# yanyan-li/PlanarSLAM

Measured on AMD Instinct MI355X. Metric: RGB-D frames/sec (extract+match+pose-opt) @640x480; 1->8-GPU batch scaling, higher is better.
Workload: dtype u8/f64

## Files before the change

### planarslam_amd/csrc/guided.hip

```cpp
#include "common.h"
#include "match_chunk.h"
#include "ref_arith.h"

namespace planar {
namespace guided {

using namespace chunk;
using ref::Pose;

enum { MODE_FRAME = 0, MODE_MAP = 1, MODE_BOW = 2, MODE_KF = 3 };

struct Args {
    planar_frame_view f;
    planar_last_frame_view last;
    planar_map_probes mp;
    float th, nn_ratio;
    int mono, check_orientation;
    int32_t* match;
    int32_t* nmatches;
    planar_keyframe_probes kf;
    float lsf;
    int n_levels, orb_dist;
};

template <int MODE>
__device__ void resolve_chunk(ChunkLds& s, int m, const Args& a, int32_t* match, int b, const float* from_angle, const float* to_angle_f,
                              const planar_keypoint* keys, const uint8_t* observed) {
    const int lane = threadIdx.x;
    volatile uint32_t* blk = s.blocked;
    for (int q = 0; q < m; q++) {
        const int id = s.pid[q];
        const int off = s.poff[q], cnt = s.poff[q + 1] - off;
        if (id < 0 || cnt == 0) continue;
        uint32_t k1 = 0xffffffffu;
        for (int base = 0; base < cnt; base += 64) {
            const uint32_t key = unblocked_key(s, off, cnt, base + lane, -1);
            k1 = min(k1, key);
        }
        k1 = wave_min_u32_shfl(k1);
        if (k1 == 0xffffffffu) continue;
        const int bestDist = (int)(k1 >> 16), bestK = (int)(k1 & 0xffff);
        const uint32_t e1 = s.cand[off + bestK];
        const int bestIdx = e1 & 0xfff, bestLevel = (e1 >> 12) & 0xf;
        int bestDist2 = 256, bestLevel2 = -1;
        if (MODE != MODE_FRAME && MODE != MODE_KF) {
            uint32_t k2 = 0xffffffffu;
            for (int base = 0; base < cnt; base += 64) {
                const uint32_t key = unblocked_key(s, off, cnt, base + lane, bestK);
                k2 = min(k2, key);
            }
            k2 = wave_min_u32_shfl(k2);
            if (k2 != 0xffffffffu) {
                bestDist2 = (int)(k2 >> 16);
                bestLevel2 = (s.cand[off + (k2 & 0xffff)] >> 12) & 0xf;
            }
        }
        bool take;
        if (MODE == MODE_FRAME) take = bestDist <= TH_HIGH;
        else if (MODE == MODE_MAP) take = bestDist <= TH_HIGH && !(bestLevel == bestLevel2 && (float)bestDist > a.nn_ratio * (float)bestDist2);
        else if (MODE == MODE_KF) take = bestDist <= a.orb_dist;
        else take = bestDist <= TH_LOW && (float)bestDist < a.nn_ratio * (float)bestDist2;
        if (!take) continue;
        if (lane == 0) {
            match[bestIdx] = id;
            const bool now_blocked = (MODE == MODE_BOW || MODE == MODE_KF) ? true : (observed[id] != 0);
            const uint32_t w = blk[bestIdx >> 5], bit = 1u << (bestIdx & 31);
            blk[bestIdx >> 5] = now_blocked ? (w | bit) : (w & ~bit);
            s.nmatches++;
            if (MODE != MODE_MAP && a.check_orientation) {
                const float to = MODE == MODE_BOW ? to_angle_f[bestIdx] : keys[bestIdx].angle;
                const int n = s.n_ev++;
                s.ev_idx[n] = (uint16_t)bestIdx;
                s.ev_bin[n] = (uint8_t)ref::rot_bin(from_angle[id], to);
            }
        }
        __builtin_amdgcn_wave_barrier();
    }
}

template <int MODE>
__global__ __launch_bounds__(NT) void projection_kernel(Args a) {
    extern __shared__ __align__(16) uint8_t lds_raw[];
    ChunkLds& s = *(ChunkLds*)lds_raw;
    const int b = blockIdx.x, tid = threadIdx.x;
    const planar_frame_view& f = a.f;
    const int N = f.n[b];
    const planar_keypoint* keys = f.keys_un + (size_t)b * f.stride;
    const float* uR = f.u_right + (size_t)b * f.stride;
    const uint8_t* desc = f.desc + (size_t)b * f.stride * 32;
    int32_t* const match_b = a.match + (size_t)b * f.stride;

    for (int w = tid; w < MAXN / 32; w += NT) s.blocked[w] = 0;
    if (tid == 0) { s.n_ev = 0; s.nmatches = 0; }
    build_grid(s, f, keys, N);
    if (f.blocked) {
        const uint8_t* bl = f.blocked + (size_t)b * f.stride;
        for (int i = tid; i < N; i += NT)
            if (bl[i]) atomicOr(&s.blocked[i >> 5], 1u << (i & 31));
    }

    Pose P;
    bool bForward = false, bBackward = false;
    size_t po;
    int NP;
    const uint8_t *probe_desc, *observed;
    if (MODE == MODE_FRAME) {
        const float* Tl = a.last.Tcw + (size_t)b * 16;
        ref::load_pose_frame(f.Tcw + (size_t)b * 16, P);
        const float tlc2 = ref::gemm_small_row_add(Tl + 8, P.Ow, Tl[11]);
        bForward = tlc2 > f.b && !a.mono;
        bBackward = -tlc2 > f.b && !a.mono;
        po = (size_t)b * a.last.stride;
        NP = a.last.n[b];
        probe_desc = a.last.mp_desc + po * 32;
        observed = a.last.mp_observed + po;
    } else if (MODE == MODE_KF) {
        ref::load_pose_frame(f.Tcw + (size_t)b * 16, P);
        po = (size_t)b * a.kf.stride;
        NP = a.kf.n[b];
        probe_desc = a.kf.desc + po * 32;
        observed = nullptr;
    } else {
        po = (size_t)b * a.mp.stride;
        NP = a.mp.n[b];
        probe_desc = a.mp.desc + po * 32;
        observed = a.mp.observed + po;
    }
    const bool bFactor = a.th != 1.0f;
    __syncthreads();

    for (int base = 0; base < NP;) {
        const int p = base + tid;
        bool valid = false;
        float u = 0, v = 0, r = 0, ur = 0;
        int minL = -1, maxL = -1;
        if (p < NP) {
            if (MODE == MODE_FRAME) {
                if (a.last.usable[po + p]) {
                    const float* xw = a.last.xw + (po + p) * 3;
                    const float xc = ref::gemm_small_row_add(P.Rcw, xw, P.tcw[0]);
                    const float yc = ref::gemm_small_row_add(P.Rcw + 3, xw, P.tcw[1]);
                    const float zc = ref::gemm_small_row_add(P.Rcw + 6, xw, P.tcw[2]);
                    const float invzc = (float)(1.0 / (double)zc);
                    if (!(invzc < 0)) {
                        u = f.fx * xc * invzc + f.cx;
                        v = f.fy * yc * invzc + f.cy;
                        if (!(u < f.min_x || u > f.max_x) && !(v < f.min_y || v > f.max_y)) {
                            const int oct = a.last.octave[po + p];
                            r = a.th * f.scale_factors[oct];
                            if (bForward) { minL = oct; maxL = -1; }
                            else if (bBackward) { minL = 0; maxL = oct; }
                            else { minL = oct - 1; maxL = oct + 1; }
                            ur = u - f.bf * invzc;
                            valid = true;
                        }
                    }
                }
            } else if (MODE == MODE_KF) {
                if (a.kf.usable[po + p] && !(a.kf.found && a.kf.found[po + p])) {
                    const float* X = a.kf.xw + (po + p) * 3;
                    const float xc = ref::gemm_small_row_add(P.Rcw, X, P.tcw[0]);
                    const float yc = ref::gemm_small_row_add(P.Rcw + 3, X, P.tcw[1]);
                    const float zc = ref::gemm_small_row_add(P.Rcw + 6, X, P.tcw[2]);
                    const float invzc = (float)(1.0 / (double)zc);
                    u = f.fx * xc * invzc + f.cx;
                    v = f.fy * yc * invzc + f.cy;
                    if (!(u < f.min_x || u > f.max_x) && !(v < f.min_y || v > f.max_y)) {
                        const float PO[3] = {X[0] - P.Ow[0], X[1] - P.Ow[1], X[2] - P.Ow[2]};
                        const float dist3D = (float)ref::norm3(PO);
                        const float maxDistance = 1.2f * a.kf.max_dist[po + p], minDistance = 0.8f * a.kf.min_dist[po + p];
                        if (!(dist3D < minDistance || dist3D > maxDistance)) {
                            const float ratio = a.kf.max_dist[po + p] / dist3D;
                            int lvl = (int)ceilf((float)log((double)ratio) / a.lsf);
                            if (lvl < 0) lvl = 0; else if (lvl >= a.n_levels) lvl = a.n_levels - 1;
                            r = a.th * f.scale_factors[lvl];
                            minL = lvl - 1; maxL = lvl + 1;
                            valid = true;
                        }
                    }
                }
            } else {
                if (a.mp.in_view[po + p]) {
                    const int lvl = a.mp.level[po + p];
                    float rr = (double)a.mp.view_cos[po + p] > 0.998 ? 2.5f : 4.0f;
                    if (bFactor) rr *= a.th;
                    r = rr * f.scale_factors[lvl];
                    u = a.mp.proj_x[po + p]; v = a.mp.proj_y[po + p]; ur = a.mp.proj_xr[po + p];
                    minL = lvl - 1; maxL = lvl;
                    valid = true;
                }
            }
        }
        int cnt = 0;
        if (valid) frame_features_in_area<MODE != MODE_KF>(s, f, keys, uR, u, v, r, minL, maxL, ur, [&](int, int) { cnt++; });
        int total;
        const int off = ref::block_exscan<NT / 64>(cnt, s.wsum, &total);
        if (tid == 0) s.m_fit = 0;
        __syncthreads();
        const bool fits = p < NP && off + cnt <= CAND_CAP;
        if (fits) atomicAdd(&s.m_fit, 1);
        s.pid[tid] = valid ? p : -1;
        s.poff[tid] = off;
        if (tid == NT - 1) s.poff[NT] = total;
        __syncthreads();
        const int m = s.m_fit;
        if (fits && valid && cnt > 0) {
            uint32_t d[8];
            ref::load_desc(d, probe_desc + (size_t)p * 32);
            int k = off;
            frame_features_in_area<MODE != MODE_KF>(s, f, keys, uR, u, v, r, minL, maxL, ur, [&](int idx, int oct) {
                const int dist = ref::hamming256(d, desc + (size_t)idx * 32);
                s.cand[k++] = ((uint32_t)dist << 16) | ((uint32_t)(oct & 0xf) << 12) | (uint32_t)idx;
            });
        }
        __syncthreads();
        const float* from_angle = MODE == MODE_FRAME ? a.last.angle + po : MODE == MODE_KF ? a.kf.angle + po : nullptr;
        if (tid < 64) resolve_chunk<MODE>(s, m, a, match_b, b, from_angle, nullptr, keys, observed);
        __syncthreads();
        base += m;
    }
    if (MODE == MODE_FRAME && a.check_orientation) rotation_filter(s, match_b);
    if (MODE == MODE_KF && a.check_orientation) rotation_filter_ranked(s, match_b);
    __syncthreads();
    if (tid == 0) a.nmatches[b] = s.nmatches;
}

struct BowArgs {
    const int32_t *n_kf, *kf_node, *n_f, *f_node;
    const uint8_t *kf_usable, *kf_desc, *f_desc;
    const float *kf_angle, *f_angle;
    int kf_stride, f_stride;
};

struct BowLds {
    ChunkLds base;
    unsigned long long kkey[MAXN], fkey[MAXN];
};

__global__ __launch_bounds__(NT) void bow_kernel(BowArgs g, Args a) {
    extern __shared__ __align__(16) uint8_t lds_raw[];
    BowLds& L = *(BowLds*)lds_raw;
    ChunkLds& s = L.base;
    const int b = blockIdx.x, tid = threadIdx.x;
    const int NK = g.n_kf[b], NF = g.n_f[b];
    const size_t ko = (size_t)b * g.kf_stride, fo = (size_t)b * g.f_stride;
    int32_t* const match_b = a.match + fo;
    for (int w = tid; w < MAXN / 32; w += NT) s.blocked[w] = 0;
    if (tid == 0) { s.n_ev = 0; s.nmatches = 0; }
    for (int i = tid; i < NF; i += NT) match_b[i] = -1;
    int pk = 1; while (pk < NK) pk <<= 1;
    int pf = 1; while (pf < NF) pf <<= 1;
    for (int i = tid; i < pk; i += NT) {
        const int node = i < NK ? g.kf_node[ko + i] : -1;
        L.kkey[i] = node >= 0 ? ((unsigned long long)node << 12) | (unsigned)i : ~0ull;
    }
    for (int i = tid; i < pf; i += NT) {
        const int node = i < NF ? g.f_node[fo + i] : -1;
        L.fkey[i] = node >= 0 ? ((unsigned long long)node << 12) | (unsigned)i : ~0ull;
    }
    bitonic_sort_u64(L.kkey, pk);
    bitonic_sort_u64(L.fkey, pf);

    for (int base = 0; base < NK;) {
        const int p = base + tid;
        bool valid = false;
        int lo = 0, hi = 0, kf = -1;
        if (p < NK && L.kkey[p] != ~0ull) {
            kf = (int)(L.kkey[p] & 0xfff);
            if (g.kf_usable[ko + kf]) {
                const unsigned long long node = L.kkey[p] >> 12;
                int x = 0, y = NF;
                while (x < y) { const int mid = (x + y) >> 1; if ((L.fkey[mid] >> 12) < node) x = mid + 1; else y = mid; }
                lo = x; y = NF;
                while (x < y) { const int mid = (x + y) >> 1; if ((L.fkey[mid] >> 12) <= node) x = mid + 1; else y = mid; }
                hi = x;
                valid = true;
            }
        }
        const int cnt = valid ? hi - lo : 0;
        int total;
        const int off = ref::block_exscan<NT / 64>(cnt, s.wsum, &total);
        if (tid == 0) s.m_fit = 0;
        __syncthreads();
        const bool fits = p < NK && off + cnt <= CAND_CAP;
        if (fits) atomicAdd(&s.m_fit, 1);
        s.pid[tid] = valid ? kf : -1;
        s.poff[tid] = off;
        if (tid == NT - 1) s.poff[NT] = total;
        __syncthreads();
        const int m = s.m_fit;
        if (fits && cnt > 0) {
            uint32_t d[8];
            ref::load_desc(d, g.kf_desc + (ko + kf) * 32);
            for (int k = 0; k < cnt; k++) {
                const int idx = (int)(L.fkey[lo + k] & 0xfff);
                const int dist = ref::hamming256(d, g.f_desc + (fo + idx) * 32);
                s.cand[off + k] = ((uint32_t)dist << 16) | (uint32_t)idx;
            }
        }
        __syncthreads();
        if (tid < 64) resolve_chunk<MODE_BOW>(s, m, a, match_b, b, g.kf_angle + ko, g.f_angle + fo, nullptr, nullptr);
        __syncthreads();
        base += m;
    }
    if (a.check_orientation) rotation_filter(s, match_b);
    __syncthreads();
    if (tid == 0) a.nmatches[b] = s.nmatches;
}

constexpr int MAX_LINES = 1024;

struct LineArgs {
    const int32_t *n_lines, *n_ml, *ml_level;
    const planar_keyline* keylines;
    const uint8_t *ldesc, *blocked, *ml_in_view, *ml_desc, *ml_observed;
    const float *ml_proj, *ml_view_cos;
    int line_stride, ml_stride;
    float scale_factors[PLANAR_MAX_LEVELS];
    float th, nn_ratio;
    int32_t *match, *nmatches;
};

__global__ __launch_bounds__(64) void lsd_projection_kernel(LineArgs a) {
    __shared__ uint32_t blocked[MAX_LINES / 32];
    const int b = blockIdx.x, lane = threadIdx.x;
    const int NLn = a.n_lines[b], NM = a.n_ml[b];
    const size_t lo = (size_t)b * a.line_stride, mo = (size_t)b * a.ml_stride;
    const planar_keyline* kl = a.keylines + lo;
    const uint8_t* ldesc = a.ldesc + lo * 32;
    int32_t* match = a.match + lo;
    volatile uint32_t* blk = blocked;
    for (int w = lane; w < MAX_LINES / 32; w += 64) blocked[w] = 0;
    __builtin_amdgcn_wave_barrier();
    if (a.blocked)
        for (int i = lane; i < NLn; i += 64)
            if (a.blocked[lo + i]) atomicOr(&blocked[i >> 5], 1u << (i & 31));
    __builtin_amdgcn_wave_barrier();
    const bool bFactor = a.th != 1.0f;
    int nmatches = 0;
    for (int j = 0; j < NM; j++) {
        if (!a.ml_in_view[mo + j]) continue;
        const int lvl = a.ml_level[mo + j];
        if (lvl < 0 || lvl >= PLANAR_MAX_LEVELS) continue;
        float r = (double)a.ml_view_cos[mo + j] > 0.998 ? 5.0f : 8.0f;
        if (bFactor) r *= a.th;
        const float* pr = a.ml_proj + (mo + j) * 4;
        const float x1 = pr[0], y1 = pr[1], x2 = pr[2], y2 = pr[3];
        const float rr = r * a.scale_factors[lvl];
        const int minLevel = lvl - 1, maxLevel = lvl;
        const bool bCheckLevels = (minLevel > 0) || (maxLevel > 0);
        uint32_t d[8];
        ref::load_desc(d, a.ml_desc + (mo + j) * 32);
        uint32_t k1 = 0xffffffffu, k2 = 0xffffffffu;
        for (int pass = 0; pass < 2; pass++) {
            uint32_t kmin = 0xffffffffu;
            for (int base = 0; base < NLn; base += 64) {
                const int i = base + lane;
                uint32_t key = 0xffffffffu;
                if (i < NLn && !(pass == 1 && i == (int)(k1 & 0xffff))) {
                    const planar_keyline k = kl[i];
                    const double mx = 0.5 * (double)(x1 + x2) - (double)k.pt_x, my = 0.5 * (double)(y1 + y2) - (double)k.pt_y;
                    const float distance = (float)(mx * mx + my * my);
                    bool ok = !(distance > rr * rr);
                    const float slope = (y1 - y2) / (x1 - x2) - k.angle;
                    if ((double)slope > (double)rr * 0.01) ok = false;
                    if (bCheckLevels) {
                        if (k.octave < minLevel) ok = false;
                        if (maxLevel >= 0 && k.octave > maxLevel) ok = false;
                    }
                    if (ok && !((blk[i >> 5] >> (i & 31)) & 1u)) key = ((uint32_t)ref::hamming256(d, ldesc + (size_t)i * 32) << 16) | (uint32_t)i;
                }
                kmin = min(kmin, key);
            }
            kmin = wave_min_u32_shfl(kmin);
            if (pass == 0) { k1 = kmin; if (k1 == 0xffffffffu) break; } else k2 = kmin;
        }
        if (k1 == 0xffffffffu) continue;
        const int bestDist = (int)(k1 >> 16), bestIdx = (int)(k1 & 0xffff);
        const int bestLevel = kl[bestIdx].octave;
        int bestDist2 = 256, bestLevel2 = -1;
        if (k2 != 0xffffffffu) { bestDist2 = (int)(k2 >> 16); bestLevel2 = kl[k2 & 0xffff].octave; }
        if (bestDist <= TH_HIGH) {
            if (bestLevel == bestLevel2 && (float)bestDist > a.nn_ratio * (float)bestDist2) continue;
            if (lane == 0) {
                match[bestIdx] = j;
                const uint32_t w = blk[bestIdx >> 5], bit = 1u << (bestIdx & 31);
                blk[bestIdx >> 5] = a.ml_observed[mo + j] ? (w | bit) : (w & ~bit);
            }
            nmatches++;
            __builtin_amdgcn_wave_barrier();
        }
    }
    if (lane == 0) a.nmatches[b] = nmatches;
}

__global__ __launch_bounds__(64) void plane_match_kernel(const int32_t* n_planes, int pl_stride, const float* pl_coef, const float* Tcw,
                                                         int map_shared, const int32_t* n_mp, int mp_stride, const uint8_t* mp_valid,
                                                         const float* mp_coef, const int32_t* mp_npts, int pts_stride, const float* mp_pts,
                                                         float dTh, float aTh, float verTh, float parTh, int32_t* match, int32_t* ver,
                                                         int32_t* par, int32_t* nmatches) {
    const int b = blockIdx.y, i = blockIdx.x, lane = threadIdx.x;
    if (i >= n_planes[b]) return;
    const int m = map_shared ? 0 : b;
    const size_t po = (size_t)b * pl_stride + i, mo = (size_t)m * mp_stride;
    const float* T = Tcw + (size_t)b * 16;
    const float* c = pl_coef + po * 4;
    float pM[4];
    for (int r = 0; r < 4; r++) {
        const float t = T[r] * c[0] + T[4 + r] * c[1] + T[8 + r] * c[2] + T[12 + r] * c[3];
        pM[r] = (float)((double)t * 1.0);
    }
    float ldTh = dTh, lverTh = verTh, lparTh = parTh;
    bool found = false;
    int im = -1, iv = -1, ip = -1;
    const int NM = n_mp[m];
    for (int j = 0; j < NM; j++) {
        if (!mp_valid[mo + j]) continue;
        const float* pW = mp_coef + (mo + j) * 4;
        const float angle = pM[0] * pW[0] + pM[1] * pW[1] + pM[2] * pW[2];
        if (angle > aTh || angle < -aTh) {
            const float* pts = mp_pts + (mo + j) * (size_t)pts_stride * 3;
            const int np = mp_npts[mo + j];
            float res = 100.0f;
            for (int k = lane; k < np; k += 64) {
                const float dis = fabsf(pM[0] * pts[3 * k] + pM[1] * pts[3 * k + 1] + pM[2] * pts[3 * k + 2] + pM[3]);
                res = fminf(res, dis);
            }
            for (int o = 32; o >= 1; o >>= 1) res = fminf(res, __shfl_xor(res, o, 64));
            if ((double)res < (double)ldTh) { ldTh = res; im = j; found = true; continue; }
        }
        if (angle < lverTh && angle > -lverTh) { lverTh = fabsf(angle); iv = j; continue; }
        if (angle > lparTh || angle < -lparTh) { lparTh = fabsf(angle); ip = j; }
    }
    if (lane == 0) {
        if (im >= 0) match[po] = im;
        if (iv >= 0) ver[po] = iv;
        if (ip >= 0) par[po] = ip;
        if (found) atomicAdd(&nmatches[b], 1);
    }
}

__global__ __launch_bounds__(256) void frustum_points_kernel(planar_frame_view F, float lsf, int n_levels, const int32_t* __restrict__ n, int stride,
                                                             const uint8_t* __restrict__ valid, const float* __restrict__ xw,
                                                             const float* __restrict__ normal, const float* __restrict__ min_dist,
                                                             const float* __restrict__ max_dist, float limit, uint8_t* __restrict__ in_view,
                                                             float* __restrict__ proj_x, float* __restrict__ proj_y, float* __restrict__ proj_xr,
                                                             int32_t* __restrict__ level, float* __restrict__ view_cos) {
    const int b = blockIdx.y, j = blockIdx.x * 256 + threadIdx.x;
    if (j >= n[b]) return;
    const size_t o = (size_t)b * stride + j;
    in_view[o] = 0;
    if (!valid[o]) return;
    Pose P;
    ref::load_pose_frame(F.Tcw + (size_t)b * 16, P);
// ... 536 lines not shown
                       d_normal, d_min_dist, d_max_dist, viewing_cos_limit, d_in_view, d_proj, d_level, d_view_cos);
    PLANAR_HIP_CHECK(hipGetLastError());
    return PLANAR_OK;
}

int planar_is_in_frustum_lines(planar_ctx* ctx, const planar_frame_view* f, float log_scale_factor, const int32_t* n, int stride, const uint8_t* valid,
                               const double* xw6, const double* normal, const float* min_dist, const float* max_dist, float viewing_cos_limit, uint8_t* in_view,
                               float* proj, int32_t* level, float* view_cos) {
    if (int rc = check_frustum_args(ctx, f, 1, stride, n && valid && xw6 && normal && min_dist && max_dist && in_view && proj && level && view_cos)) return rc;
    PLANAR_HIP_CHECK(hipSetDevice(ctx->device));
    Stager s;
    planar_frame_view d = *f;
    const size_t B = (size_t)f->B, N = B * stride;
    s.in_field(d.Tcw, B * 16);
    const auto d_n = s.in(n, B);
    const auto d_valid = s.in(valid, N);
    const auto d_xw6 = s.in(xw6, N * 6), d_normal = s.in(normal, N * 3);
    const auto d_min = s.in(min_dist, N), d_max = s.in(max_dist, N);
    const auto d_in_view = s.inout(in_view, N);
    const auto d_proj = s.inout(proj, N * 4);
    const auto d_level = s.inout(level, N);
    const auto d_cos = s.inout(view_cos, N);
    return s.run(ctx->stream, [&] {
        return planar_is_in_frustum_lines_dev(ctx, &d, log_scale_factor, d_n, stride, d_valid, d_xw6, d_normal, d_min, d_max, viewing_cos_limit, d_in_view, d_proj, d_level, d_cos);
    });
}

int planar_search_by_bow_dev(planar_ctx* ctx, int B, const int32_t* d_n_kf, int kf_stride, const int32_t* d_kf_node, const uint8_t* d_kf_usable,
                             const float* d_kf_angle, const uint8_t* d_kf_desc, const int32_t* d_n_f, int f_stride, const int32_t* d_f_node,
                             const float* d_f_angle, const uint8_t* d_f_desc, float nn_ratio, int check_orientation, int32_t* d_match,
                             int32_t* d_nmatches) {
    if (int rc = check_bow_args(ctx, B, kf_stride, f_stride, d_n_kf && d_kf_node && d_kf_usable && d_kf_angle && d_kf_desc && d_n_f && d_f_node && d_f_angle && d_f_desc && d_match &&
                                                                 d_nmatches))
        return rc;
    static bool attr_set = false;
    if (!attr_set) {
        PLANAR_HIP_CHECK(hipFuncSetAttribute((const void*)guided::bow_kernel, hipFuncAttributeMaxDynamicSharedMemorySize, (int)sizeof(guided::BowLds)));
        attr_set = true;
    }
    guided::BowArgs g{d_n_kf, d_kf_node, d_n_f, d_f_node, d_kf_usable, d_kf_desc, d_f_desc, d_kf_angle, d_f_angle, kf_stride, f_stride};
    Args a{};
    a.nn_ratio = nn_ratio; a.check_orientation = check_orientation; a.match = d_match; a.nmatches = d_nmatches;
    hipLaunchKernelGGL(guided::bow_kernel, dim3(B), dim3(guided::NT), sizeof(guided::BowLds), ctx->stream, g, a);
    PLANAR_HIP_CHECK(hipGetLastError());
    return PLANAR_OK;
}

int planar_search_by_bow(planar_ctx* ctx, int B, const int32_t* n_kf, int kf_stride, const int32_t* kf_node, const uint8_t* kf_usable,
                         const float* kf_angle, const uint8_t* kf_desc, const int32_t* n_f, int f_stride, const int32_t* f_node,
                         const float* f_angle, const uint8_t* f_desc, float nn_ratio, int check_orientation, int32_t* match, int32_t* nmatches) {
    if (int rc = check_bow_args(ctx, B, kf_stride, f_stride, n_kf && kf_node && kf_usable && kf_angle && kf_desc && n_f && f_node && f_angle && f_desc && match && nmatches)) return rc;
    PLANAR_HIP_CHECK(hipSetDevice(ctx->device));
    Stager s;
    const size_t nb = (size_t)B, nk = nb * kf_stride, nf = nb * f_stride;
    const auto d_n_kf = s.in(n_kf, nb), d_kf_node = s.in(kf_node, nk);
    const auto d_kf_usable = s.in(kf_usable, nk);
    const auto d_kf_angle = s.in(kf_angle, nk);
    const auto d_kf_desc = s.in(kf_desc, nk * 32);
    const auto d_n_f = s.in(n_f, nb), d_f_node = s.in(f_node, nf);
    const auto d_f_angle = s.in(f_angle, nf);
    const auto d_f_desc = s.in(f_desc, nf * 32);
    const auto d_match = s.inout(match, nf), d_n = s.out(nmatches, nb);
    return s.run(ctx->stream, [&] {
        return planar_search_by_bow_dev(ctx, B, d_n_kf, kf_stride, d_kf_node, d_kf_usable, d_kf_angle, d_kf_desc, d_n_f, f_stride, d_f_node, d_f_angle, d_f_desc, nn_ratio,
                                        check_orientation, d_match, d_n);
    });
}

int planar_lsd_search_by_projection_dev(planar_ctx* ctx, int B, const int32_t* d_n_lines, int line_stride, const planar_keyline* d_keylines,
                                        const uint8_t* d_ldesc, const uint8_t* d_blocked, const int32_t* d_n_ml, int ml_stride,
                                        const uint8_t* d_ml_in_view, const float* d_ml_proj, const int32_t* d_ml_level, const float* d_ml_view_cos,
                                        const uint8_t* d_ml_desc, const uint8_t* d_ml_observed, const float* scale_factors, int n_levels, float th,
                                        float nn_ratio, int32_t* d_match, int32_t* d_nmatches) {
    if (int rc = check_lsd_projection_args(ctx, B, line_stride, ml_stride, n_levels, d_n_lines && d_keylines && d_ldesc && d_n_ml && d_ml_in_view && d_ml_proj && d_ml_level &&
                                                                                         d_ml_view_cos && d_ml_desc && d_ml_observed && scale_factors && d_match && d_nmatches))
        return rc;
    guided::LineArgs a{};
    a.n_lines = d_n_lines; a.n_ml = d_n_ml; a.ml_level = d_ml_level; a.keylines = d_keylines; a.ldesc = d_ldesc; a.blocked = d_blocked;
    a.ml_in_view = d_ml_in_view; a.ml_desc = d_ml_desc; a.ml_observed = d_ml_observed; a.ml_proj = d_ml_proj; a.ml_view_cos = d_ml_view_cos;
    a.line_stride = line_stride; a.ml_stride = ml_stride; a.th = th; a.nn_ratio = nn_ratio; a.match = d_match; a.nmatches = d_nmatches;
    for (int i = 0; i < n_levels; i++) a.scale_factors[i] = scale_factors[i];
    hipLaunchKernelGGL(guided::lsd_projection_kernel, dim3(B), dim3(64), 0, ctx->stream, a);
    PLANAR_HIP_CHECK(hipGetLastError());
    return PLANAR_OK;
}

int planar_lsd_search_by_projection(planar_ctx* ctx, int B, const int32_t* n_lines, int line_stride, const planar_keyline* keylines,
                                    const uint8_t* ldesc, const uint8_t* blocked, const int32_t* n_ml, int ml_stride, const uint8_t* ml_in_view,
                                    const float* ml_proj, const int32_t* ml_level, const float* ml_view_cos, const uint8_t* ml_desc,
                                    const uint8_t* ml_observed, const float* scale_factors, int n_levels, float th, float nn_ratio, int32_t* match,
                                    int32_t* nmatches) {
    if (int rc = check_lsd_projection_args(ctx, B, line_stride, ml_stride, n_levels, n_lines && keylines && ldesc && n_ml && ml_in_view && ml_proj && ml_level && ml_view_cos &&
                                                                                         ml_desc && ml_observed && scale_factors && match && nmatches))
        return rc;
    PLANAR_HIP_CHECK(hipSetDevice(ctx->device));
    Stager s;
    const size_t nb = (size_t)B, nl = nb * line_stride, nm = nb * ml_stride;
    const auto d_n_lines = s.in(n_lines, nb);
    const auto d_keylines = s.in(keylines, nl);
    const auto d_ldesc = s.in(ldesc, nl * 32), d_blocked = s.in(blocked, nl);
    const auto d_n_ml = s.in(n_ml, nb);
    const auto d_in_view = s.in(ml_in_view, nm);
    const auto d_proj = s.in(ml_proj, nm * 4);
    const auto d_level = s.in(ml_level, nm);
    const auto d_cos = s.in(ml_view_cos, nm);
    const auto d_desc = s.in(ml_desc, nm * 32), d_observed = s.in(ml_observed, nm);
    const auto d_match = s.inout(match, nl), d_n = s.out(nmatches, nb);
    return s.run(ctx->stream, [&] {
        return planar_lsd_search_by_projection_dev(ctx, B, d_n_lines, line_stride, d_keylines, d_ldesc, d_blocked, d_n_ml, ml_stride, d_in_view, d_proj, d_level, d_cos, d_desc,
                                                   d_observed, scale_factors, n_levels, th, nn_ratio, d_match, d_n);
    });
}

int planar_plane_search_by_coefficients_dev(planar_ctx* ctx, int B, const int32_t* d_n_planes, int pl_stride, const float* d_pl_coef,
                                            const float* d_Tcw, int map_shared, const int32_t* d_n_mp, int mp_stride, const uint8_t* d_mp_valid,
                                            const float* d_mp_coef, const int32_t* d_mp_npts, int pts_stride, const float* d_mp_pts, const float* th,
                                            int32_t* d_match, int32_t* d_ver, int32_t* d_par, int32_t* d_nmatches) {
    if (int rc = check_plane_search_args(ctx, B, pl_stride, mp_stride, pts_stride, d_n_planes && d_pl_coef && d_Tcw && d_n_mp && d_mp_valid && d_mp_coef && d_mp_npts && d_mp_pts && th &&
                                                                                       d_match && d_ver && d_par && d_nmatches))
        return rc;
    PLANAR_HIP_CHECK(hipMemsetAsync(d_nmatches, 0, (size_t)B * 4, ctx->stream));
    hipLaunchKernelGGL(guided::plane_match_kernel, dim3(pl_stride, B), dim3(64), 0, ctx->stream, d_n_planes, pl_stride, d_pl_coef, d_Tcw, map_shared,
                       d_n_mp, mp_stride, d_mp_valid, d_mp_coef, d_mp_npts, pts_stride, d_mp_pts, th[0], th[1], th[2], th[3], d_match, d_ver, d_par,
                       d_nmatches);
    PLANAR_HIP_CHECK(hipGetLastError());
    return PLANAR_OK;
}

int planar_plane_search_by_coefficients(planar_ctx* ctx, int B, const int32_t* n_planes, int pl_stride, const float* pl_coef, const float* Tcw,
                                        int map_shared, const int32_t* n_mp, int mp_stride, const uint8_t* mp_valid, const float* mp_coef,
                                        const int32_t* mp_npts, int pts_stride, const float* mp_pts, const float* th, int32_t* match, int32_t* ver,
                                        int32_t* par, int32_t* nmatches) {
    if (int rc = check_plane_search_args(ctx, B, pl_stride, mp_stride, pts_stride, n_planes && pl_coef && Tcw && n_mp && mp_valid && mp_coef && mp_npts && mp_pts && th && match && ver &&
                                                                                       par && nmatches))
        return rc;
    PLANAR_HIP_CHECK(hipSetDevice(ctx->device));
    Stager s;
    const size_t nb = (size_t)B, MB = map_shared ? 1 : nb, np = nb * pl_stride, nm = MB * mp_stride;
    const auto d_n_planes = s.in(n_planes, nb);
    const auto d_pl_coef = s.in(pl_coef, np * 4), d_Tcw = s.in(Tcw, nb * 16);
    const auto d_n_mp = s.in(n_mp, MB);
    const auto d_mp_valid = s.in(mp_valid, nm);
    const auto d_mp_coef = s.in(mp_coef, nm * 4);
    const auto d_mp_npts = s.in(mp_npts, nm);
    const auto d_mp_pts = s.in(mp_pts, nm * pts_stride * 3);
    const auto d_match = s.inout(match, np), d_ver = s.inout(ver, np), d_par = s.inout(par, np), d_n = s.out(nmatches, nb);
    return s.run(ctx->stream, [&] {
        return planar_plane_search_by_coefficients_dev(ctx, B, d_n_planes, pl_stride, d_pl_coef, d_Tcw, map_shared, d_n_mp, mp_stride, d_mp_valid, d_mp_coef, d_mp_npts, pts_stride,
                                                       d_mp_pts, th, d_match, d_ver, d_par, d_n);
    });
}

}
```

### planarslam_amd/csrc/match_chunk.h

```cpp
#pragma once
#include "common.h"
#include "ref_arith.h"

namespace planar {
namespace chunk {

using ref::HISTO_LENGTH;

constexpr int NT = 256;
constexpr int NCELL = PLANAR_GRID_COLS * PLANAR_GRID_ROWS;
constexpr int MAXN = PLANAR_MAX_FRAME_KEYS;
constexpr int CAND_CAP = 8192;
constexpr int TH_HIGH = 100, TH_LOW = 50;

struct ChunkLds {
    uint32_t cand[CAND_CAP];
    uint16_t cell_start[NCELL + 1];
    uint16_t items[MAXN];
    uint32_t blocked[MAXN / 32];
    int pid[NT];
    int poff[NT + 1];
    uint16_t ev_idx[MAXN];
    uint8_t ev_bin[MAXN];
    int hist[HISTO_LENGTH];
    int keep[3];
    int n_ev, nmatches, m_fit, wsum[NT / 64];
};

__device__ inline uint32_t wave_min_u32_shfl(uint32_t v) {
    for (int o = 32; o >= 1; o >>= 1) v = min(v, (uint32_t)__shfl_xor((int)v, o, 64));
    return v;
}

template <typename L>
__device__ void build_grid(L& s, const planar_frame_view& f, const planar_keypoint* keys, int N) {
    const int tid = threadIdx.x;
    uint32_t* cnt = s.cand;
    for (int c = tid; c < NCELL; c += NT) cnt[c] = 0;
    __syncthreads();
    for (int i = tid; i < N; i += NT) {
        const int px = (int)roundf((keys[i].x - f.min_x) * f.grid_w_inv);
        const int py = (int)roundf((keys[i].y - f.min_y) * f.grid_h_inv);
        if (px < 0 || px >= PLANAR_GRID_COLS || py < 0 || py >= PLANAR_GRID_ROWS) continue;
        atomicAdd(&cnt[px * PLANAR_GRID_ROWS + py], 1u);
    }
    __syncthreads();
    constexpr int PER = NCELL / NT;
    int local = 0;
    for (int k = 0; k < PER; k++) local += (int)cnt[tid * PER + k];
    int total;
    int run = ref::block_exscan<NT / 64>(local, s.wsum, &total);
    for (int k = 0; k < PER; k++) {
        const int c = tid * PER + k, n = (int)cnt[c];
        s.cell_start[c] = (uint16_t)run;
        cnt[c] = (uint32_t)run;
        run += n;
    }
    if (tid == NT - 1) s.cell_start[NCELL] = (uint16_t)run;
    __syncthreads();
    for (int i = tid; i < N; i += NT) {
        const int px = (int)roundf((keys[i].x - f.min_x) * f.grid_w_inv);
        const int py = (int)roundf((keys[i].y - f.min_y) * f.grid_h_inv);
        if (px < 0 || px >= PLANAR_GRID_COLS || py < 0 || py >= PLANAR_GRID_ROWS) continue;
        const uint32_t pos = atomicAdd(&cnt[px * PLANAR_GRID_ROWS + py], 1u);
        s.items[pos] = (uint16_t)i;
    }
    __syncthreads();
    for (int k = 0; k < PER; k++) {
        const int c = tid * PER + k;
        const int a = s.cell_start[c], e = s.cell_start[c + 1];
        for (int i = a + 1; i < e; i++) {
            const uint16_t v = s.items[i];
            int j = i - 1;
            while (j >= a && s.items[j] > v) { s.items[j + 1] = s.items[j]; j--; }
            s.items[j + 1] = v;
        }
    }
    __syncthreads();
}

template <bool STEREO = true, typename L, typename Emit>
__device__ inline void frame_features_in_area(const L& s, const planar_frame_view& f, const planar_keypoint* keys, const float* uR, float x, float y,
                                              float r, int minLevel, int maxLevel, float ur, Emit emit) {
    const int nMinCellX = max(0, (int)floorf((x - f.min_x - r) * f.grid_w_inv));
    if (nMinCellX >= PLANAR_GRID_COLS) return;
    const int nMaxCellX = min(PLANAR_GRID_COLS - 1, (int)ceilf((x - f.min_x + r) * f.grid_w_inv));
    if (nMaxCellX < 0) return;
    const int nMinCellY = max(0, (int)floorf((y - f.min_y - r) * f.grid_h_inv));
    if (nMinCellY >= PLANAR_GRID_ROWS) return;
    const int nMaxCellY = min(PLANAR_GRID_ROWS - 1, (int)ceilf((y - f.min_y + r) * f.grid_h_inv));
    if (nMaxCellY < 0) return;
    const bool bCheckLevels = (minLevel > 0) || (maxLevel >= 0);
    for (int ix = nMinCellX; ix <= nMaxCellX; ix++) {
        if (nMinCellY > nMaxCellY) break;
        const int a = s.cell_start[ix * PLANAR_GRID_ROWS + nMinCellY], e = s.cell_start[ix * PLANAR_GRID_ROWS + nMaxCellY + 1];
        for (int k = a; k < e; k++) {
            const int idx = s.items[k];
            const planar_keypoint kp = keys[idx];
            if (bCheckLevels) {
                if (kp.octave < minLevel) continue;
                if (maxLevel >= 0 && kp.octave > maxLevel) continue;
            }
            const float distx = kp.x - x, disty = kp.y - y;
            if (!(fabsf(distx) < r && fabsf(disty) < r)) continue;
            if (STEREO) {
                const float u2 = uR[idx];
                if (u2 > 0) {
                    const float er = fabsf(ur - u2);
                    if (er > r) continue;
                }
            }
            emit(idx, kp.octave);
        }
    }
}

template <typename L, typename Emit>
__device__ inline void keyframe_features_in_area(const L& s, const planar_frame_view& f, const planar_keypoint* keys, float u, float v, float radius, int lvl,
                                                 Emit emit) {
    const int nMinCellX = max(0, (int)floorf((u - f.min_x - radius) * f.grid_w_inv));
    const int nMaxCellX = min(PLANAR_GRID_COLS - 1, (int)ceilf((u - f.min_x + radius) * f.grid_w_inv));
    const int nMinCellY = max(0, (int)floorf((v - f.min_y - radius) * f.grid_h_inv));
    const int nMaxCellY = min(PLANAR_GRID_ROWS - 1, (int)ceilf((v - f.min_y + radius) * f.grid_h_inv));
    if (!(nMinCellX < PLANAR_GRID_COLS && nMaxCellX >= 0 && nMinCellY < PLANAR_GRID_ROWS && nMaxCellY >= 0 && nMinCellY <= nMaxCellY)) return;
    for (int ix = nMinCellX; ix <= nMaxCellX; ix++) {
        const int c0 = s.cell_start[ix * PLANAR_GRID_ROWS + nMinCellY], c1 = s.cell_start[ix * PLANAR_GRID_ROWS + nMaxCellY + 1];
        for (int k = c0; k < c1; k++) {
            const int idx = s.items[k];
            const planar_keypoint kp = keys[idx];
            if (!(fabsf(kp.x - u) < radius && fabsf(kp.y - v) < radius)) continue;
            if (kp.octave < lvl - 1 || kp.octave > lvl) continue;
            emit(idx);
        }
    }
}

__device__ inline uint32_t unblocked_key(const ChunkLds& s, int off, int cnt, int k, int skip) {
    const volatile uint32_t* blk = s.blocked;
    uint32_t key = 0xffffffffu;
    if (k < cnt && k != skip) {
        const uint32_t e = s.cand[off + k];
        const int idx = e & 0xfff;
        if (!((blk[idx >> 5] >> (idx & 31)) & 1u)) key = ((e >> 16) << 16) | (uint32_t)k;
    }
    return key;
}

__device__ void rotation_filter(ChunkLds& s, int32_t* match) {
    const int tid = threadIdx.x;
    if (tid < HISTO_LENGTH) s.hist[tid] = 0;
    __syncthreads();
    const int n = s.n_ev;
    for (int i = tid; i < n; i += NT) atomicAdd(&s.hist[s.ev_bin[i]], 1);
    __syncthreads();
    if (tid == 0) {
        int i1, i2, i3;
        ref::three_maxima(s.hist, i1, i2, i3);
        s.keep[0] = i1; s.keep[1] = i2; s.keep[2] = i3;
        int removed = 0;
        for (int i = 0; i < HISTO_LENGTH; i++)
            if (i != i1 && i != i2 && i != i3) removed += s.hist[i];
        s.nmatches -= removed;
    }
    __syncthreads();
    const int k1 = s.keep[0], k2 = s.keep[1], k3 = s.keep[2];
    for (int i = tid; i < n; i += NT) {
        const int bin = s.ev_bin[i];
        if (bin != k1 && bin != k2 && bin != k3) match[s.ev_idx[i]] = -1;
    }
}

__device__ void rotation_filter_ranked(ChunkLds& s, int32_t* match) {
    const int tid = threadIdx.x;
    if (tid < HISTO_LENGTH) s.hist[tid] = 0;
    if (tid < 3) s.keep[tid] = -1;
    __syncthreads();
    const int n = s.n_ev;
    for (int i = tid; i < n; i += NT) atomicAdd(&s.hist[s.ev_bin[i]], 1);
    __syncthreads();
    if (tid < HISTO_LENGTH && s.hist[tid] > 0) {
        const int h = s.hist[tid];
        int rank = 0;
        for (int j = 0; j < HISTO_LENGTH; j++) { const int hj = s.hist[j]; rank += (hj > h || (hj == h && j < tid)) ? 1 : 0; }
        if (rank < 3) s.keep[rank] = tid;
    }
    __syncthreads();
    if (tid == 0) {
        const int i1 = s.keep[0], i2 = s.keep[1], i3 = s.keep[2];
        const int max1 = i1 >= 0 ? s.hist[i1] : 0, max2 = i2 >= 0 ? s.hist[i2] : 0, max3 = i3 >= 0 ? s.hist[i3] : 0;
        const bool k2 = !((float)max2 < 0.1f * (float)max1), k3 = k2 && !((float)max3 < 0.1f * (float)max1);
        if (!k2) s.keep[1] = -1;
        if (!k3) s.keep[2] = -1;
        s.nmatches -= n - (max1 + (k2 ? max2 : 0) + (k3 ? max3 : 0));
    }
    __syncthreads();
    const int k1 = s.keep[0], k2 = s.keep[1], k3 = s.keep[2];
    for (int i = tid; i < n; i += NT) {
        const int bin = s.ev_bin[i];
        if (bin != k1 && bin != k2 && bin != k3) match[s.ev_idx[i]] = -1;
    }
}

__device__ void bitonic_sort_u64(unsigned long long* key, int n_pow2) {
    for (int k = 2; k <= n_pow2; k <<= 1)
        for (int j = k >> 1; j > 0; j >>= 1) {
            __syncthreads();
            for (int i = threadIdx.x; i < n_pow2; i += NT) {
                const int ixj = i ^ j;
                if (ixj > i) {
                    const unsigned long long x = key[i], y = key[ixj];
                    const bool up = (i & k) == 0;
                    if ((x > y) == up) { key[i] = y; key[ixj] = x; }
                }
            }
        }
    __syncthreads();
}


}
}
```

Measured before the change: 12640.

## Resolve match chunks speculatively across the whole block with conflict-claim rounds

Adds a speculative parallel resolver in which every probe thread scans its own candidate list, claims its best keypoint with atomicMin, and commits the longest conflict-free prefix each round. The sequential single-wave resolve_chunk is kept only as a fallback when a list exceeds SPEC_MAX_LIST or LDS has no room for the claim array. The aim is to remove the serial per-probe resolution bottleneck in the projection and BoW matching kernels, at the cost of extra barriers per round and possibly many rounds when probes conflict heavily. It also inlines the rotation-filter three-maxima search and adds optional, compile-time-gated timing instrumentation.

```diff
diff --git a/planarslam_amd/csrc/guided.hip b/planarslam_amd/csrc/guided.hip
--- a/planarslam_amd/csrc/guided.hip
+++ b/planarslam_amd/csrc/guided.hip
@@ -9,6 +9,27 @@
 using ref::Pose;
 
 enum { MODE_FRAME = 0, MODE_MAP = 1, MODE_BOW = 2, MODE_KF = 3 };
+
+enum { SPLIT_GRID = 0, SPLIT_COUNT, SPLIT_FILL, SPLIT_RESOLVE, SPLIT_ROTATION, SPLIT_FRAMES, SPLIT_CHUNKS, SPLIT_ROUNDS, SPLIT_SERIAL_CHUNKS, SPLIT_N };
+#ifdef PLANAR_GUIDED_SPLIT
+__device__ unsigned long long g_split[4][SPLIT_N];
+struct SplitClock {
+    unsigned long long t, acc[SPLIT_N] = {};
+    __device__ SplitClock() : t(wall_clock64()) {}
+    __device__ void mark(int bucket) { const unsigned long long n = wall_clock64(); acc[bucket] += n - t; t = n; }
+    __device__ void add(int bucket, int v) { acc[bucket] += (unsigned long long)v; }
+    __device__ void flush(int mode) {
+        if (threadIdx.x == 0)
+            for (int i = 0; i < SPLIT_N; i++) atomicAdd(&g_split[mode][i], acc[i]);
+    }
+};
+#else
+struct SplitClock {
+    __device__ void mark(int) {}
+    __device__ void add(int, int) {}
+    __device__ void flush(int) {}
+};
+#endif
 
 struct Args {
     planar_frame_view f;
@@ -79,6 +100,73 @@
 }
 
 template <int MODE>
+__device__ int resolve_chunk_spec(ChunkLds& s, int m, int nkeys, const Args& a, int32_t* match, const float* from_angle, const float* to_angle_f,
+                                  const planar_keypoint* keys, const uint8_t* observed) {
+    const int q = threadIdx.x;
+    uint32_t* const claim = spec_claims(s, nkeys);
+    const int id = q < m ? s.pid[q] : -1;
+    const int off = s.poff[q], cnt = id >= 0 ? s.poff[q + 1] - off : 0;
+    bool open = cnt > 0;
+    int rounds = 0;
+    for (int start = 0; start < m; rounds++) {
+        if (q == 0) s.m_fit = m;
+        bool take = false;
+        int bestIdx = -1, secondIdx = -1;
+        if (open) {
+            uint32_t k1, k2;
+            spec_scan<MODE != MODE_FRAME && MODE != MODE_KF>(s, off, cnt, k1, k2);
+            if (k1 != 0xffffffffu) {
+                const int bestDist = (int)(k1 >> 16);
+                const uint32_t e1 = s.cand[off + (k1 & 0xffff)];
+                const int bestLevel = (e1 >> 12) & 0xf;
+                bestIdx = e1 & 0xfff;
+                int bestDist2 = 256, bestLevel2 = -1;
+                if (k2 != 0xffffffffu) {
+                    const uint32_t e2 = s.cand[off + (k2 & 0xffff)];
+                    bestDist2 = (int)(k2 >> 16);
+                    bestLevel2 = (e2 >> 12) & 0xf;
+                    secondIdx = e2 & 0xfff;
+                }
+                if (MODE == MODE_FRAME) take = bestDist <= TH_HIGH;
+                else if (MODE == MODE_MAP) take = bestDist <= TH_HIGH && !(bestLevel == bestLevel2 && (float)bestDist > a.nn_ratio * (float)bestDist2);
+                else if (MODE == MODE_KF) take = bestDist <= a.orb_dist;
+                else take = bestDist <= TH_LOW && (float)bestDist < a.nn_ratio * (float)bestDist2;
+                if (take) atomicMin(&claim[bestIdx], (uint32_t)q);
+            }
+        }
+        __syncthreads();
+        if (open) {
+            bool conflict;
+            if (SPEC_WHOLE_LIST) conflict = spec_conflict(s, claim, off, cnt, q);
+            else if (MODE == MODE_FRAME || MODE == MODE_KF) conflict = take && claim[bestIdx] < (uint32_t)q;
+            else conflict = (bestIdx >= 0 && claim[bestIdx] < (uint32_t)q) || (secondIdx >= 0 && claim[secondIdx] < (uint32_t)q);
+            if (conflict) atomicMin(&s.m_fit, q);
+        }
+        __syncthreads();
+        const int c = s.m_fit;
+        if (take) claim[bestIdx] = 0xffffffffu;
+        if (open && q < c) {
+            open = false;
+            if (take) {
+                match[bestIdx] = id;
+                const bool now_blocked = (MODE == MODE_BOW || MODE == MODE_KF) ? true : (observed[id] != 0);
+                if (now_blocked) atomicOr(&s.blocked[bestIdx >> 5], 1u << (bestIdx & 31));
+                atomicAdd(&s.nmatches, 1);
+                if (MODE != MODE_MAP && a.check_orientation) {
+                    const float to = MODE == MODE_BOW ? to_angle_f[bestIdx] : keys[bestIdx].angle;
+                    const int n = atomicAdd(&s.n_ev, 1);
+                    s.ev_idx[n] = (uint16_t)bestIdx;
+                    s.ev_bin[n] = (uint8_t)ref::rot_bin(from_angle[id], to);
+                }
+            }
+        }
+        __syncthreads();
+        start = c;
+    }
+    return rounds;
+}
+
+template <int MODE>
 __global__ __launch_bounds__(NT) void projection_kernel(Args a) {
     extern __shared__ __align__(16) uint8_t lds_raw[];
     ChunkLds& s = *(ChunkLds*)lds_raw;
@@ -90,6 +178,7 @@
     const uint8_t* desc = f.desc + (size_t)b * f.stride * 32;
     int32_t* const match_b = a.match + (size_t)b * f.stride;
 
+    SplitClock clk;
     for (int w = tid; w < MAXN / 32; w += NT) s.blocked[w] = 0;
     if (tid == 0) { s.n_ev = 0; s.nmatches = 0; }
     build_grid(s, f, keys, N);
@@ -128,6 +217,7 @@
     }
     const bool bFactor = a.th != 1.0f;
     __syncthreads();
+    clk.mark(SPLIT_GRID);
 
     for (int base = 0; base < NP;) {
         const int p = base + tid;
@@ -195,15 +285,20 @@
         if (valid) frame_features_in_area<MODE != MODE_KF>(s, f, keys, uR, u, v, r, minL, maxL, ur, [&](int, int) { cnt++; });
         int total;
         const int off = ref::block_exscan<NT / 64>(cnt, s.wsum, &total);
-        if (tid == 0) s.m_fit = 0;
+        if (tid == 0) { s.m_fit = 0; s.keep[0] = 0; }
         __syncthreads();
         const bool fits = p < NP && off + cnt <= CAND_CAP;
         if (fits) atomicAdd(&s.m_fit, 1);
+        if (fits && cnt > SPEC_MAX_LIST) s.keep[0] = 1;
         s.pid[tid] = valid ? p : -1;
         s.poff[tid] = off;
         if (tid == NT - 1) s.poff[NT] = total;
         __syncthreads();
         const int m = s.m_fit;
+        const bool spec = s.keep[0] == 0 && spec_room(s, m, N);
+        clk.mark(SPLIT_COUNT);
+        if (spec)
+            for (int i = tid; i < N; i += NT) spec_claims(s, N)[i] = 0xffffffffu;
         if (fits && valid && cnt > 0) {
             uint32_t d[8];
             ref::load_desc(d, probe_desc + (size_t)p * 32);
@@ -214,15 +309,23 @@
             });
         }
         __syncthreads();
+        clk.mark(SPLIT_FILL);
         const float* from_angle = MODE == MODE_FRAME ? a.last.angle + po : MODE == MODE_KF ? a.kf.angle + po : nullptr;
-        if (tid < 64) resolve_chunk<MODE>(s, m, a, match_b, b, from_angle, nullptr, keys, observed);
+        if (spec) clk.add(SPLIT_ROUNDS, resolve_chunk_spec<MODE>(s, m, N, a, match_b, from_angle, nullptr, keys, observed));
+        else if (tid < 64) resolve_chunk<MODE>(s, m, a, match_b, b, from_angle, nullptr, keys, observed);
         __syncthreads();
+        clk.mark(SPLIT_RESOLVE);
+        clk.add(SPLIT_CHUNKS, 1);
+        clk.add(SPLIT_SERIAL_CHUNKS, spec ? 0 : 1);
         base += m;
     }
     if (MODE == MODE_FRAME && a.check_orientation) rotation_filter(s, match_b);
     if (MODE == MODE_KF && a.check_orientation) rotation_filter_ranked(s, match_b);
     __syncthreads();
     if (tid == 0) a.nmatches[b] = s.nmatches;
+    clk.mark(SPLIT_ROTATION);
+    clk.add(SPLIT_FRAMES, 1);
+    clk.flush(MODE);
 }
 
 struct BowArgs {
@@ -236,6 +339,9 @@
     ChunkLds base;
     unsigned long long kkey[MAXN], fkey[MAXN];
 };
+
+static_assert(sizeof(ChunkLds) == 62120, "projection_kernel: two workgroups per CU");
+static_assert(sizeof(BowLds) == 127656, "bow_kernel: one workgroup per CU");
 
 __global__ __launch_bounds__(NT) void bow_kernel(BowArgs g, Args a) {
     extern __shared__ __align__(16) uint8_t lds_raw[];
@@ -280,15 +386,19 @@
         const int cnt = valid ? hi - lo : 0;
         int total;
         const int off = ref::block_exscan<NT / 64>(cnt, s.wsum, &total);
-        if (tid == 0) s.m_fit = 0;
+        if (tid == 0) { s.m_fit = 0; s.keep[0] = 0; }
         __syncthreads();
         const bool fits = p < NK && off + cnt <= CAND_CAP;
         if (fits) atomicAdd(&s.m_fit, 1);
+        if (fits && cnt > SPEC_MAX_LIST) s.keep[0] = 1;
         s.pid[tid] = valid ? kf : -1;
         s.poff[tid] = off;
         if (tid == NT - 1) s.poff[NT] = total;
         __syncthreads();
         const int m = s.m_fit;
+        const bool spec = s.keep[0] == 0 && spec_room(s, m, NF);
+        if (spec)
+            for (int i = tid; i < NF; i += NT) spec_claims(s, NF)[i] = 0xffffffffu;
         if (fits && cnt > 0) {
             uint32_t d[8];
             ref::load_desc(d, g.kf_desc + (ko + kf) * 32);
@@ -299,7 +409,8 @@
             }
         }
         __syncthreads();
-        if (tid < 64) resolve_chunk<MODE_BOW>(s, m, a, match_b, b, g.kf_angle + ko, g.f_angle + fo, nullptr, nullptr);
+        if (spec) resolve_chunk_spec<MODE_BOW>(s, m, NF, a, match_b, g.kf_angle + ko, g.f_angle + fo, nullptr, nullptr);
+        else if (tid < 64) resolve_chunk<MODE_BOW>(s, m, a, match_b, b, g.kf_angle + ko, g.f_angle + fo, nullptr, nullptr);
         __syncthreads();
         base += m;
     }
@@ -1142,3 +1253,12 @@
 }
 
 }
+
+#ifdef PLANAR_GUIDED_SPLIT
+extern "C" int planar_guided_split_read(unsigned long long* out, int reset) {
+    static const unsigned long long zero[4][guided::SPLIT_N] = {};
+    if (out) PLANAR_HIP_CHECK(hipMemcpyFromSymbol(out, HIP_SYMBOL(guided::g_split), sizeof(zero)));
+    if (reset) PLANAR_HIP_CHECK(hipMemcpyToSymbol(HIP_SYMBOL(guided::g_split), zero, sizeof(zero)));
+    return PLANAR_OK;
+}
+#endif
diff --git a/planarslam_amd/csrc/match_chunk.h b/planarslam_amd/csrc/match_chunk.h
--- a/planarslam_amd/csrc/match_chunk.h
+++ b/planarslam_amd/csrc/match_chunk.h
@@ -12,6 +12,14 @@
 constexpr int MAXN = PLANAR_MAX_FRAME_KEYS;
 constexpr int CAND_CAP = 8192;
 constexpr int TH_HIGH = 100, TH_LOW = 50;
+#ifndef PLANAR_SPEC_MAX_LIST
+#define PLANAR_SPEC_MAX_LIST 64
+#endif
+constexpr int SPEC_MAX_LIST = PLANAR_SPEC_MAX_LIST;
+#ifndef PLANAR_SPEC_WHOLE_LIST
+#define PLANAR_SPEC_WHOLE_LIST 0
+#endif
+constexpr bool SPEC_WHOLE_LIST = PLANAR_SPEC_WHOLE_LIST != 0;
 
 struct ChunkLds {
     uint32_t cand[CAND_CAP];
@@ -146,6 +154,27 @@
     return key;
 }
 
+__device__ inline uint32_t* spec_claims(ChunkLds& s, int nkeys) { return s.cand + (CAND_CAP - nkeys); }
+__device__ inline bool spec_room(const ChunkLds& s, int m, int nkeys) { return s.poff[m] + nkeys <= CAND_CAP; }
+
+template <bool SECOND>
+__device__ inline void spec_scan(const ChunkLds& s, int off, int cnt, uint32_t& k1, uint32_t& k2) {
+    k1 = k2 = 0xffffffffu;
+    for (int k = 0; k < cnt; k++) {
+        const uint32_t e = s.cand[off + k];
+        const int idx = e & 0xfff;
+        const uint32_t key = ((s.blocked[idx >> 5] >> (idx & 31)) & 1u) ? 0xffffffffu : (e & 0xffff0000u) | (uint32_t)k;
+        if (SECOND) k2 = min(k2, max(k1, key));
+        k1 = min(k1, key);
+    }
+}
+
+__device__ inline bool spec_conflict(const ChunkLds& s, const uint32_t* claim, int off, int cnt, int q) {
+    bool hit = false;
+    for (int k = 0; k < cnt; k++) hit |= claim[s.cand[off + k] & 0xfff] < (uint32_t)q;
+    return hit;
+}
+
 __device__ void rotation_filter(ChunkLds& s, int32_t* match) {
     const int tid = threadIdx.x;
     if (tid < HISTO_LENGTH) s.hist[tid] = 0;
@@ -154,8 +183,17 @@
     for (int i = tid; i < n; i += NT) atomicAdd(&s.hist[s.ev_bin[i]], 1);
     __syncthreads();
     if (tid == 0) {
-        int i1, i2, i3;
-        ref::three_maxima(s.hist, i1, i2, i3);
+        int max1 = 0, max2 = 0, max3 = 0, i1 = -1, i2 = -1, i3 = -1;
+#pragma unroll 1
+        for (int i = 0; i < HISTO_LENGTH; i++) {
+            const int sz = s.hist[i];
+            const bool g1 = sz > max1, g2 = sz > max2, g3 = sz > max3;
+            i3 = g2 ? i2 : g3 ? i : i3;    max3 = g2 ? max2 : g3 ? sz : max3;
+            i2 = g1 ? i1 : g2 ? i : i2;    max2 = g1 ? max1 : g2 ? sz : max2;
+            i1 = g1 ? i : i1;              max1 = g1 ? sz : max1;
+        }
+        if ((float)max2 < 0.1f * (float)max1) { i2 = -1; i3 = -1; }
+        else if ((float)max3 < 0.1f * (float)max1) i3 = -1;
         s.keep[0] = i1; s.keep[1] = i2; s.keep[2] = i3;
         int removed = 0;
         for (int i = 0; i < HISTO_LENGTH; i++)
```

After: 12840 (median of 6 runs). 1.02x the previous value.
